# westlake-repl/IDvs.MoRec

Hardware: AMD Instinct MI355X
Metric: user-sequences/sec end-to-end train step, SASRec+BERT-base (higher is better)
Workload: dtype fp16

## Files before the change

### idvs/morec_amd/csrc/gemm8p.hip

```cpp
#include <mutex>
#include "gemm8p_core.hpp"
#include "gemm_args.hpp"
#include "ce_args.hpp"

namespace {
using namespace g8;
constexpr int SLICE = 4096;
constexpr int LDS_TOTAL = LDS_BYTES + 8 * SLICE;

#define G8_STAMPW(i, w)                                                                                  \
    do {                                                                                                 \
        if (p.stamps && threadIdx.x == 0) p.stamps[(size_t)(w) * 16 + (i)] = __builtin_readcyclecounter(); \
    } while (0)

struct TileXY {
    int wg, m0, n0;
    int k0, nkt, tail, chunk;
    int krem;
};

template <typename TI, typename TO, int ACT, bool CS, int TMR = 256>
__device__ __forceinline__ void tile_body(const GemmArgs& p, char* smem, const bf16* __restrict__ Acur, const bf16* __restrict__ Bcur,
                                          const bf16* __restrict__ Anext, const bf16* __restrict__ Bnext, const TileXY cur, const TileXY nxt,
                                          const bool first) {
    constexpr bool PART = TMR != TM;
    constexpr int tmr = TMR;
    constexpr int nb1 = (TMR - 128) / 32;
    constexpr int ES = (int)sizeof(TO);
    constexpr int EPV = 16 / ES;
    constexpr int PC = 128 / ES;
    constexpr int NPASS = 64 / PC;
    constexpr int NG = PC / 8;
    struct Vecs { u32x4_t q[4]; };
    const int m0 = cur.m0, n0 = cur.n0;
    G8_STAMPW(0, cur.wg);
    f32x16_t acc[4][2];
    float bias_l;
    {
        int tid_m = threadIdx.x;
        asm volatile("" : "+v"(tid_m));
        {
            const float* bp = p.bias ? p.bias : reinterpret_cast<const float*>(p.B);
            bias_l = bp[min(n0 + ((tid_m >> 6) & 3) * 64 + (tid_m & 63), p.N - 1)];
        }
        Ctx c;
        make_ctx(c, tid_m, Acur, Bcur, min(p.M - m0, tmr), p.N - n0, p.lda, p.ldb, cur.krem);
        if (first) issue_prologue(c, smem, cur.nkt);
        constexpr int NST = 16 * (int)sizeof(TO) / 2;
        const int younger = (first || (p.debug & 3) || (p.debug & 64)) ? 0 : (p.aux_out ? 2 * NST : NST);
        const int wr_m = __builtin_amdgcn_readfirstlane(tid_m >> 8);
        unsigned long long* st_m = p.stamps ? p.stamps + (size_t)cur.wg * 16 : nullptr;
        if constexpr (!PART) {
            mainloop8p<TI>(c, wr_m, cur.nkt, younger, smem, acc, st_m);
        } else {
            (void)younger;
            if (wr_m == 0) mainloop8p_s<TI, 0, 0, 4>(c, 0, cur.nkt, smem, acc, st_m);
            else mainloop8p_s<TI, 0, 0, nb1>(c, 1, cur.nkt, smem, acc, st_m);
        }
    }
    G8_STAMPW(1, cur.wg);
    if (cur.tail >= 0) {
        int tid_t = threadIdx.x;
        asm volatile("" : "+v"(tid_t));
        const __amdgpu_buffer_rsrc_t rw = __builtin_amdgcn_make_buffer_rsrc((void*)(p.tail_ws + (size_t)(cur.tail * 2 + cur.chunk) * (TM * TN)), 0,
                                                                            TM * TN * 4, 0x00020000);
#pragma unroll
        for (int i = 0; i < 4; ++i)
#pragma unroll
            for (int j = 0; j < 2; ++j)
#pragma unroll
                for (int g = 0; g < 4; ++g) {
                    u32x4_t v;
#pragma unroll
                    for (int e = 0; e < 4; ++e) v[e] = __float_as_uint(acc[i][j][4 * g + e]);
                    __builtin_amdgcn_raw_buffer_store_b128(v, rw, tid_t * 16, ((i * 2 + j) * 4 + g) * (THREADS * 16), 16);
                }
        vm_wait<0>();
        __syncthreads();
        int* flag = reinterpret_cast<int*>(smem + LDS_BYTES);
        if (threadIdx.x == 0) *flag = __hip_atomic_fetch_add(p.tail_cnt + cur.tail, 1, __ATOMIC_RELAXED, __HIP_MEMORY_SCOPE_AGENT);
        __syncthreads();
        const int ticket = __builtin_amdgcn_readfirstlane(*flag);
        __syncthreads();
        if (ticket == 0) return;
        if (threadIdx.x == 0) __hip_atomic_store(p.tail_cnt + cur.tail, 0, __ATOMIC_RELAXED, __HIP_MEMORY_SCOPE_AGENT);
        const __amdgpu_buffer_rsrc_t rr = __builtin_amdgcn_make_buffer_rsrc((void*)(p.tail_ws + (size_t)(cur.tail * 2 + (cur.chunk ^ 1)) * (TM * TN)), 0,
                                                                            TM * TN * 4, 0x00020000);
#pragma unroll
        for (int i = 0; i < 4; ++i) {
            u32x4_t v[2][4];
#pragma unroll
            for (int j = 0; j < 2; ++j)
#pragma unroll
                for (int g = 0; g < 4; ++g) v[j][g] = __builtin_amdgcn_raw_buffer_load_b128(rr, tid_t * 16, ((i * 2 + j) * 4 + g) * (THREADS * 16), 16);
#pragma unroll
            for (int j = 0; j < 2; ++j)
#pragma unroll
                for (int g = 0; g < 4; ++g)
#pragma unroll
                    for (int e = 0; e < 4; ++e) acc[i][j][4 * g + e] += __uint_as_float(v[j][g][e]);
            pin();
        }
    }
    int tid_e = threadIdx.x;
    asm volatile("" : "+v"(tid_e));
    const int lane = tid_e & 63, r5 = lane & 31, h = lane >> 5;
    const int wave = __builtin_amdgcn_readfirstlane(tid_e >> 6);
    const int wr = wave >> 2, wc = wave & 3;
    char* ws = smem + LDS_BYTES + wave * SLICE;
    TO* C = reinterpret_cast<TO*>(p.C);
    TO* aux = reinterpret_cast<TO*>(p.aux_out);
    const TO* din = reinterpret_cast<const TO*>(p.dact_in);
    auto wfence = [&]() {
        __builtin_amdgcn_fence(__ATOMIC_RELEASE, "wavefront");
        __builtin_amdgcn_wave_barrier();
        __builtin_amdgcn_fence(__ATOMIC_ACQUIRE, "wavefront");
    };
    const int rs_row = lane >> 3, rs_slot = lane & 7;
    const int rs_off = rs_row * 128 + ((rs_slot ^ (rs_row & 7)) << 4);
    auto cell = [&](int q) {
        const int slot = ES == 2 ? q : 2 * q + h;
        return reinterpret_cast<TO*>(ws + r5 * 128 + ((slot ^ (r5 & 7)) << 4) + (ES == 2 ? 8 * h : 0));
    };
    const int cur_tm = m0 / tmr;
    const int mw = m0 + wr * 128, nw = n0 + wc * 64;
    const int m_end = min(p.M, m0 + tmr);
    const int nblk = (PART && wr) ? nb1 : 4;
    const long tile_bytes = (long)min(tmr, p.M - m0) * p.ldc * ES;
    const int ext = (int)min(tile_bytes, 0x7fffffffL);
    const size_t tile_off = (size_t)m0 * p.ldc;
    const __amdgpu_buffer_rsrc_t rC = __builtin_amdgcn_make_buffer_rsrc((void*)(C + tile_off), 0, ext, 0x00020000);
    const __amdgpu_buffer_rsrc_t rD = __builtin_amdgcn_make_buffer_rsrc((void*)(((ACT >= 3) ? din : C) + tile_off), 0, ext, 0x00020000);
    auto lane_off = [&](int ps) {
        const int n = nw + ps * PC + rs_slot * EPV;
        return n < p.N ? (uint32_t)((rs_row * p.ldc + n) * ES) : 0x80000000u;
    };
    auto row_term = [&](int Mi, int i) { return (uint32_t)((wr * 128 + Mi * 32 + 8 * i) * p.ldc * ES); };
    auto rows_store = [&](const __amdgpu_buffer_rsrc_t& rs, int Mi, uint32_t lo) {
        u32x4_t q[4];
#pragma unroll
        for (int i = 0; i < 4; ++i) q[i] = *reinterpret_cast<const u32x4_t*>(ws + rs_off + i * 1024);
        if (!(p.debug & 1)) {
            const int cp = (p.debug >> 4) & 3;
            if (cp == 0) {
#pragma unroll
                for (int i = 0; i < 4; ++i) __builtin_amdgcn_raw_buffer_store_b128(q[i], rs, lo + row_term(Mi, i), 0, 0);
            } else if (cp == 1) {
#pragma unroll
                for (int i = 0; i < 4; ++i) __builtin_amdgcn_raw_buffer_store_b128(q[i], rs, lo + row_term(Mi, i), 0, 2);
            } else if (cp == 2) {
#pragma unroll
                for (int i = 0; i < 4; ++i) __builtin_amdgcn_raw_buffer_store_b128(q[i], rs, lo + row_term(Mi, i), 0, 16);
            } else {
#pragma unroll
                for (int i = 0; i < 4; ++i) __builtin_amdgcn_raw_buffer_store_b128(q[i], rs, lo + row_term(Mi, i), 0, 18);
            }
        }
    };
    auto rows_fetch = [&](const __amdgpu_buffer_rsrc_t& rs, int Mi, uint32_t lo) {
        Vecs r;
#pragma unroll
        for (int i = 0; i < 4; ++i) r.q[i] = __builtin_amdgcn_raw_buffer_load_b128(rs, lo + row_term(Mi, i), 0, 0);
        return r;
    };
    auto rows_put = [&](const Vecs r) {
#pragma unroll
        for (int i = 0; i < 4; ++i) *reinterpret_cast<u32x4_t*>(ws + rs_off + i * 1024) = r.q[i];
    };
    uint32_t lo[NPASS];
#pragma unroll
    for (int ps = 0; ps < NPASS; ++ps) lo[ps] = lane_off(ps);

    float4 bv[2][4];
    if constexpr (ACT < 3) {
        reinterpret_cast<float*>(ws)[lane] = p.bias ? bias_l : 0.f;
        wfence();
#pragma unroll
        for (int Ni = 0; Ni < 2; ++Ni)
#pragma unroll
            for (int g = 0; g < 4; ++g) bv[Ni][g] = *reinterpret_cast<const float4*>(ws + (Ni * 32 + g * 8 + 4 * h) * 4);
        wfence();
    } else {
#pragma unroll
        for (int Ni = 0; Ni < 2; ++Ni)
#pragma unroll
            for (int g = 0; g < 4; ++g) bv[Ni][g] = make_float4(0.f, 0.f, 0.f, 0.f);
    }
    Vecs dq[2] = {Vecs(), Vecs()};
    if constexpr (ACT >= 3) {
        dq[0] = rows_fetch(rD, 0, lo[0]);
        dq[1] = rows_fetch(rD, 1 / NPASS, lo[1 % NPASS]);
    }
    pin();

    {
        int tid_n = threadIdx.x;
        asm volatile("" : "+v"(tid_n));
        Ctx cn;
        make_ctx(cn, tid_n, Anext, Bnext, min(p.M - nxt.m0, tmr), p.N - nxt.n0, p.lda, p.ldb, nxt.krem);
        issue_prologue(cn, smem, nxt.nkt);
    }
    if (p.debug & 2) {
        if (acc[0][0][0] == 12345.678f) reinterpret_cast<float*>(p.C)[0] = acc[1][1][3] + acc[2][0][7] + acc[3][1][15] + bv[0][0].x;
        return;
    }
    if (p.stamps) { asm volatile("" :: "v"(bv[0][0].x), "v"(bv[1][3].w)); G8_STAMPW(2, cur.wg); }
    [[maybe_unused]] float cs8[8] = {0.f, 0.f, 0.f, 0.f, 0.f, 0.f, 0.f, 0.f};
#pragma unroll
    for (int Mi = 0; Mi < 4; ++Mi) {
        if constexpr (PART) {
            if (Mi >= nblk) break;
        }
        [[maybe_unused]] const bool row_ok = (mw + Mi * 32 + r5) < m_end;
#pragma unroll
        for (int ps = 0; ps < NPASS; ++ps) {
            pin();
            if constexpr (ACT >= 3) {
                constexpr int LAST = 4 * NPASS - 1;
                const int it = Mi * NPASS + ps, nx = it + 2;
                rows_put(dq[it & 1]);
                if (nx <= LAST) dq[it & 1] = rows_fetch(rD, nx / NPASS, lo[nx % NPASS]);
                wfence();
            }
            if (aux) {
                if constexpr (ACT == 1 || ACT == 2) {
                    static_assert(ES == 2, "activation epilogues are instantiated for bf16 outputs");
                    uint2 park[NG];
#pragma unroll
                    for (int q = 0; q < NG; ++q) {
                        const int Ni = q / 4, g = q % 4;
                        const float4 b = bv[Ni][g];
                        float v[4], d[4];
                        v[0] = fmaf(acc[Mi][Ni][4 * g + 0], p.alpha, b.x);
                        v[1] = fmaf(acc[Mi][Ni][4 * g + 1], p.alpha, b.y);
                        v[2] = fmaf(acc[Mi][Ni][4 * g + 2], p.alpha, b.z);
                        v[3] = fmaf(acc[Mi][Ni][4 * g + 3], p.alpha, b.w);
#pragma unroll
                        for (int r = 0; r < 4; ++r) d[r] = v[r];
                        if (p.aux_deriv) {
                            if constexpr (ACT == 1) {
                                gelu4_with_deriv(v, d);
                            } else {
#pragma unroll
                                for (int r = 0; r < 4; ++r) { d[r] = v[r] > 0.f ? 1.f : 0.f; v[r] = fmaxf(v[r], 0.f); }
                            }
                        } else {
                            if constexpr (ACT == 1) {
                                gelu4(v);
                            } else {
#pragma unroll
                                for (int r = 0; r < 4; ++r) v[r] = fmaxf(v[r], 0.f);
                            }
                        }
                        io<TO>::store4(cell(q), d);
                        park[q] = make_uint2(h16<TI>::pack2(v[0], v[1]), h16<TI>::pack2(v[2], v[3]));
                        if (q & 1) pin();
                    }
                    wfence();
                    rows_store(__builtin_amdgcn_make_buffer_rsrc((void*)(aux + tile_off), 0, ext, 0x00020000), Mi, lo[ps]);
                    wfence();
#pragma unroll
                    for (int q = 0; q < NG; ++q) *reinterpret_cast<uint2*>(cell(q)) = park[q];
                    wfence();
                    rows_store(rC, Mi, lo[ps]);
                    wfence();
                    continue;
                } else {
#pragma unroll
                    for (int q = 0; q < NG; ++q) {
                        const int Ni = ES == 2 ? q / 4 : ps, g = ES == 2 ? q % 4 : q;
                        const float4 b = bv[Ni][g];
                        float pre[4];
                        pre[0] = fmaf(acc[Mi][Ni][4 * g + 0], p.alpha, b.x);
                        pre[1] = fmaf(acc[Mi][Ni][4 * g + 1], p.alpha, b.y);
                        pre[2] = fmaf(acc[Mi][Ni][4 * g + 2], p.alpha, b.z);
                        pre[3] = fmaf(acc[Mi][Ni][4 * g + 3], p.alpha, b.w);
                        io<TO>::store4(cell(q), pre);
                        if (q & 1) pin();
                    }
                    wfence();
                    rows_store(__builtin_amdgcn_make_buffer_rsrc((void*)(aux + tile_off), 0, ext, 0x00020000), Mi, lo[ps]);
                    wfence();
                }
            }
            [[maybe_unused]] uint32_t uraw[NG][ES == 2 ? 2 : 4];
            if constexpr (ACT >= 3) {
#pragma unroll
                for (int q = 0; q < NG; ++q) {
                    if constexpr (ES == 2) {
                        const uint2 t = *reinterpret_cast<const uint2*>(cell(q));
                        uraw[q][0] = t.x; uraw[q][1] = t.y;
                    } else {
                        const uint4 t = *reinterpret_cast<const uint4*>(cell(q));
                        uraw[q][0] = t.x; uraw[q][1] = t.y; uraw[q][2] = t.z; uraw[q][3] = t.w;
                    }
                }
            }
#pragma unroll
            for (int q = 0; q < NG; ++q) {
                const int Ni = ES == 2 ? q / 4 : ps, g = ES == 2 ? q % 4 : q;
                const float4 b = bv[Ni][g];
                float v[4];
                v[0] = fmaf(acc[Mi][Ni][4 * g + 0], p.alpha, b.x);
                v[1] = fmaf(acc[Mi][Ni][4 * g + 1], p.alpha, b.y);
                v[2] = fmaf(acc[Mi][Ni][4 * g + 2], p.alpha, b.z);
                v[3] = fmaf(acc[Mi][Ni][4 * g + 3], p.alpha, b.w);
                if constexpr (ACT == 1) {
                    gelu4(v);
                } else if constexpr (ACT == 2) {
#pragma unroll
                    for (int r = 0; r < 4; ++r) v[r] = fmaxf(v[r], 0.f);
                } else if constexpr (ACT >= 3) {
                    float u[4];
                    if constexpr (ES == 2) {
                        u[0] = h16<TI>::bits2f(uraw[q][0] & 0xffffu); u[1] = h16<TI>::bits2f(uraw[q][0] >> 16);
                        u[2] = h16<TI>::bits2f(uraw[q][1] & 0xffffu); u[3] = h16<TI>::bits2f(uraw[q][1] >> 16);
                    } else {
#pragma unroll
                        for (int r = 0; r < 4; ++r) u[r] = __uint_as_float(uraw[q][r]);
                    }
                    if constexpr (ACT == 3) {
                        dgelu4_mul(v, u);
                    } else if constexpr (ACT == 4) {
#pragma unroll
                        for (int r = 0; r < 4; ++r) v[r] = (u[r] > 0.f) ? v[r] : 0.f;
                    } else {
#pragma unroll
                        for (int r = 0; r < 4; ++r) v[r] *= u[r];
                    }
                }
                if constexpr (CS) {
#pragma unroll
                    for (int r = 0; r < 4; ++r) v[r] = row_ok ? v[r] : 0.f;
                }
                io<TO>::store4(cell(q), v);
                if (ACT != 5 && (q & 1)) pin();
            }
            wfence();
            if constexpr (CS) {
                static_assert(!CS || ES == 2, "fused column sums: bf16 output only");
                u32x4_t q[4];
#pragma unroll
                for (int i = 0; i < 4; ++i) q[i] = *reinterpret_cast<const u32x4_t*>(ws + rs_off + i * 1024);
#pragma unroll
                for (int i = 0; i < 4; ++i)
#pragma unroll
                    for (int w = 0; w < 4; ++w) {
                        cs8[2 * w] += h16<TI>::bits2f(q[i][w] & 0xffffu);
                        cs8[2 * w + 1] += h16<TI>::bits2f(q[i][w] >> 16);
                    }
                if (!(p.debug & 1)) {
#pragma unroll
                    for (int i = 0; i < 4; ++i) __builtin_amdgcn_raw_buffer_store_b128(q[i], rC, lo[ps] + row_term(Mi, i), 0, 0);
                }
            } else {
                rows_store(rC, Mi, lo[ps]);
            }
            wfence();
        }
        G8_STAMPW(3 + Mi, cur.wg);
    }
    G8_STAMPW(7, cur.wg);
    if constexpr (CS) {
#pragma unroll
        for (int j = 0; j < 8; ++j) {
            cs8[j] += __shfl_xor(cs8[j], 8, 64);
            cs8[j] += __shfl_xor(cs8[j], 16, 64);
            cs8[j] += __shfl_xor(cs8[j], 32, 64);
        }
        if (rs_row == 0) {
            const int n = nw + rs_slot * 8;
            float* dst = p.colsum + (size_t)(cur_tm * 2 + wr) * p.N + n;
#pragma unroll
            for (int j = 0; j < 8; ++j)
                if (n + j < p.N) dst[j] = cs8[j];
        }
    }
}

template <typename TI, typename TO, int ACT, bool CS, int TMR = 256>
__global__ __launch_bounds__(THREADS) void gemm8p_kernel(GemmArgs p) {
    extern __shared__ __attribute__((aligned(16))) char smem[];
    const int nwg = p.tiles_m * p.tiles_n;
    const bf16* A = reinterpret_cast<const bf16*>(p.A);
    const bf16* B = reinterpret_cast<const bf16*>(p.B);
    const int Keff = (p.debug & 4) ? 128 : p.K;
    const int nk = (Keff + KE - 1) / KE;
    const int krem_all = Keff - (nk - 1) * KE;
    const int G = gridDim.x, F = nwg / G, R = nwg - F * G;
    const bool split = p.tail_ws != nullptr && F >= 1 && R >= 1 && 2 * R <= G && nk >= 24;
    const int nk0 = (nk + p.tail_bias) / 2;
    const int n_units = F + ((int)blockIdx.x < (split ? 2 * R : R) ? 1 : 0);
    auto unit_at = [&](int i) {
        TileXY t;
        int vb = (int)blockIdx.x + i * G;
        t.k0 = 0; t.nkt = nk; t.tail = -1; t.chunk = 0; t.krem = krem_all;
        if (i >= F && split) {
            t.chunk = (int)blockIdx.x >= R ? 1 : 0;
            t.tail = (int)blockIdx.x - t.chunk * R;
            vb = F * G + t.tail;
            t.k0 = t.chunk ? nk0 : 0;
            t.nkt = t.chunk ? nk - nk0 : nk0;
            t.krem = t.chunk ? krem_all : KE;
        }
        t.wg = xcd_remap(vb, nwg);
        int tm, tn;
        if (p.ngroup <= 0 || p.ngroup >= p.tiles_n) {
            tm = t.wg / p.tiles_n;
            tn = t.wg % p.tiles_n;
        } else {
            const int per = p.ngroup * p.tiles_m, ng = (p.tiles_n + p.ngroup - 1) / p.ngroup;
            const int g = min(t.wg / per, ng - 1), r = t.wg - g * per;
            const int w = g == ng - 1 ? p.tiles_n - g * p.ngroup : p.ngroup;
            tm = r / w;
            tn = g * p.ngroup + r % w;
        }
        t.m0 = tm * TMR;
        t.n0 = tn * TN;
        return t;
    };
    TileXY cur = unit_at(0);
    if (p.debug >> 8) {
        const int GS = (p.debug >> 8) & 0xff;
        const long long T = (long long)nk * 2300 + 9000;
        const long long until = (long long)__builtin_readcyclecounter() + T * ((blockIdx.x >> 3) % GS) / GS;
        while ((long long)__builtin_readcyclecounter() < until) __builtin_amdgcn_s_sleep(16);
    }
    for (int i = 0; i < n_units; ++i) {
        const bool more = i + 1 < n_units;
        const TileXY nxt = more ? unit_at(i + 1) : cur;
        tile_body<TI, TO, ACT, CS, TMR>(p, smem, A + (size_t)cur.m0 * p.lda + cur.k0 * KE, B + (size_t)cur.n0 * p.ldb + cur.k0 * KE,
                               A + (size_t)nxt.m0 * p.lda + nxt.k0 * KE, B + (size_t)nxt.n0 * p.ldb + nxt.k0 * KE, cur, nxt, i == 0);
        cur = nxt;
    }
    vm_wait<0>();
}

static void tail_workspace(hipStream_t s, int n_cu, GemmArgs& a) {
    struct Slot { hipStream_t s; float* ws; int* cnt; int dev; };
    static Slot slots[8];
    static int n_slots = 0;
    static std::mutex mu;
    std::lock_guard<std::mutex> lock(mu);
    int dev = 0;
    (void)hipGetDevice(&dev);
    for (int i = 0; i < n_slots; ++i)
        if (slots[i].s == s && slots[i].dev == dev) { a.tail_ws = slots[i].ws; a.tail_cnt = slots[i].cnt; return; }
    if (n_slots == 8) return;
    const size_t ws_bytes = (size_t)n_cu * TM * TN * sizeof(float), cnt_bytes = (size_t)n_cu * sizeof(int);
    char* base = nullptr;
    if (hipMalloc(reinterpret_cast<void**>(&base), ws_bytes + cnt_bytes) != hipSuccess) { (void)hipGetLastError(); return; }
    if (hipMemset(base + ws_bytes, 0, cnt_bytes) != hipSuccess) { (void)hipGetLastError(); (void)hipFree(base); return; }
    slots[n_slots] = Slot{s, reinterpret_cast<float*>(base), reinterpret_cast<int*>(base + ws_bytes), dev};
    a.tail_ws = slots[n_slots].ws;
    a.tail_cnt = slots[n_slots].cnt;
    ++n_slots;
}

static_assert(TM == gplan::P8_TM && TN == gplan::P8_TN && KE == gplan::P8_KE, "gemm_plan.hpp");

template <typename TI, typename TO, int ACT, bool CS, int TMR = 256>
int launch8p(const GemmPlan& p, GemmArgs& a, hipStream_t s) {
    a.tmr = TMR;
    a.tiles_m = (a.M + TMR - 1) / TMR;
    a.tiles_n = (a.N + TN - 1) / TN;
    static const hipError_t attr_rc = hipFuncSetAttribute(reinterpret_cast<const void*>(&gemm8p_kernel<TI, TO, ACT, CS, TMR>),
                                                          hipFuncAttributeMaxDynamicSharedMemorySize, LDS_TOTAL);
    (void)attr_rc;
    const int n_cu = p.n_cu;
    const int nwg = a.tiles_m * a.tiles_n;
    a.ngroup = p.ngroup;
    a.tail_ws = nullptr;
    a.tail_cnt = nullptr;
    if (p.tail_split) tail_workspace(s, n_cu, a);
    hipLaunchKernelGGL((gemm8p_kernel<TI, TO, ACT, CS, TMR>), dim3(nwg < n_cu ? nwg : n_cu), dim3(THREADS), LDS_TOTAL, s, a);
    MOREC_CHECK_LAUNCH();
    if constexpr (CS) return colsum_f32_launch(a.colsum, a.colsum_dst, a.tiles_m * 2, a.N, s);
    return MOREC_OK;
}

template <typename TI>
int dispatch8p(const GemmPlan& p, GemmArgs& a, hipStream_t s) {
    const int mode = p.mode;
    if (p.tile_rows == 224) {
        if (mode == 0) return launch8p<TI, TI, 0, false, 224>(p, a, s);
        if (mode == 1) return launch8p<TI, TI, 1, false, 224>(p, a, s);
        return launch8p<TI, TI, 5, true, 224>(p, a, s);
    }
    if (p.tile_rows == 192) {
        if (mode == 0) return launch8p<TI, TI, 0, false, 192>(p, a, s);
        if (mode == 1) return launch8p<TI, TI, 1, false, 192>(p, a, s);
        return launch8p<TI, TI, 5, true, 192>(p, a, s);
    }
    if (p.out_dtype == MOREC_F32) return launch8p<TI, float, 0, false>(p, a, s);
    if (p.colsum) {
        if (mode == 3) return launch8p<TI, TI, 3, true>(p, a, s);
        if (mode == 4) return launch8p<TI, TI, 4, true>(p, a, s);
        return launch8p<TI, TI, 5, true>(p, a, s);
    }
    switch (mode) {
        case 1: return launch8p<TI, TI, 1, false>(p, a, s);
        case 2: return launch8p<TI, TI, 2, false>(p, a, s);
        case 3: return launch8p<TI, TI, 3, false>(p, a, s);
        case 4: return launch8p<TI, TI, 4, false>(p, a, s);
        case 5: return launch8p<TI, TI, 5, false>(p, a, s);
        default: return launch8p<TI, TI, 0, false>(p, a, s);
    }
}
}

int gemm8p_launch(const GemmPlan& p, GemmArgs& a, hipStream_t s) {
    const Tuning& t = tuning();
    a.debug = t.gemm8p_debug;
    a.tail_bias = t.gemm8p_tail_bias;
    a.tail_split = t.gemm8p_tail_split;
    a.stamps = reinterpret_cast<unsigned long long*>(t.gemm8p_stamps());
    return p.in_dtype == MOREC_F16 ? dispatch8p<f16>(p, a, s) : dispatch8p<bf16>(p, a, s);
}
```

### idvs/morec_amd/csrc/gemm8p_core.hpp

```cpp
#pragma once
#include "gemm_core.hpp"

namespace g8 {
typedef f32x16c_t f32x16_t;
typedef __attribute__((ext_vector_type(4))) unsigned int u32x4_t;

constexpr int TM = 256, TN = 256, KE = 64;
constexpr int KB = 128;
constexpr int OP_BYTES = 256 * KB;
constexpr int BUF_BYTES = 2 * OP_BYTES;
constexpr int LDS_BYTES = 2 * BUF_BYTES;
constexpr int THREADS = 512;

template <int N>
__device__ __forceinline__ void vm_wait() {
    asm volatile("s_waitcnt vmcnt(%0)" ::"n"(N) : "memory");
}
__device__ __forceinline__ void pin() { __builtin_amdgcn_sched_barrier(0); }
__device__ __forceinline__ void bar() {
    pin();
    __builtin_amdgcn_s_barrier();
    pin();
}

typedef __attribute__((address_space(8))) void* rsrc_t;

template <int AUX = 0>
__device__ __forceinline__ void dma2(__amdgpu_buffer_rsrc_t rs, uint32_t o0, uint32_t o1, int kbyte, char* dst) {
    __builtin_amdgcn_raw_ptr_buffer_load_lds(rs, (lptr_t)dst, 16, o0, kbyte, 0, AUX);
    __builtin_amdgcn_raw_ptr_buffer_load_lds(rs, (lptr_t)(dst + 1024), 16, o1, kbyte, 0, AUX);
}
struct Ctx;
template <int AUX = 0>
__device__ __forceinline__ void dma2z(__amdgpu_buffer_rsrc_t rs, uint32_t o0, uint32_t o1, const uint32_t (&pz)[2], uint32_t m, int kbyte, char* dst) {
    dma2<AUX>(rs, o0 | (pz[0] & m), o1 | (pz[1] & m), kbyte, dst);
}

struct Ctx {
    __amdgpu_buffer_rsrc_t ra, rb;
    uint32_t a1[2], a2[2], b1[2], b2[2];
    int dA1, dA2, dB1, dB2;
    int aoff, boff;
    int loff[4];
    uint32_t pz[2];
};

__device__ __forceinline__ uint4 lds16(const char* p) { return *reinterpret_cast<const uint4*>(p); }

template <typename T16, int M0, int NQ, bool ZERO, int NBW = 4>
__device__ __forceinline__ void mfma_quadrant(f32x16_t (&acc)[4][2], const uint4 (&fa)[2][4], const uint4 (&fb)[4]) {
    if constexpr (M0 >= NBW) return;
    constexpr int NMI = (M0 + 1 < NBW) ? 2 : 1;
#ifndef G8_NO_SETPRIO
    __builtin_amdgcn_s_setprio(1);
#endif
#pragma unroll
    for (int ks = 0; ks < 4; ++ks)
#pragma unroll
        for (int mi = 0; mi < NMI; ++mi) {
            f32x16_t cin = acc[M0 + mi][NQ];
            if constexpr (ZERO) {
                if (ks == 0) {
#pragma unroll
                    for (int v = 0; v < 16; ++v) cin[v] = 0.f;
                }
            }
            acc[M0 + mi][NQ] = h16<T16>::mma32(__builtin_bit_cast(bf16x8_t, fb[ks]), __builtin_bit_cast(bf16x8_t, fa[mi][ks]), cin);
        }
#ifndef G8_NO_SETPRIO
    __builtin_amdgcn_s_setprio(0);
#endif
}

template <int REM, int W1, int W0, int SLACK = 0>
__device__ __forceinline__ void vm_wait_tail() {
    vm_wait<(REM >= 2 ? 8 + SLACK : (REM == 1 ? W1 : W0))>();
}

#ifdef G8_EXP_SHADOW
#define G8_GS_PARAM , float (&gs)[4]
#define G8_GS_ARG , gs
#ifndef G8_EXP_SHADOW_MASK
#define G8_EXP_SHADOW_MASK 15
#endif
#define G8_SHADOW() G8_SHADOW_P(0)
#define G8_SHADOW_P(ph_)                                              \
    do {                                                              \
        if (!((G8_EXP_SHADOW_MASK >> (ph_)) & 1)) break;              \
        pin();                                                        \
        _Pragma("unroll") for (int u_ = 0; u_ < G8_EXP_SHADOW; ++u_) { \
            float d_[4];                                              \
            gelu4_with_deriv(gs, d_);                                 \
            _Pragma("unroll") for (int r_ = 0; r_ < 4; ++r_) gs[r_] = gs[r_] * 0.5f + d_[r_]; \
        }                                                             \
        pin();                                                        \
    } while (0)
#else
#define G8_GS_PARAM
#define G8_GS_ARG
#define G8_SHADOW() do {} while (0)
#define G8_SHADOW_P(ph_) do {} while (0)
#endif
template <typename T16, int REM, int SLACK = 0, bool ZERO = false, int BAUX = 0, int NBW = 4>
__device__ __forceinline__ void ktile(char* smem, const Ctx& c, int cb, int kb, f32x16_t (&acc)[4][2], bool last2 G8_GS_PARAM) {
    const uint32_t m1 = REM == 1 ? 0xffffffffu : 0u;
    const uint32_t m2 = last2 ? 0xffffffffu : 0u;
    static_assert(SLACK == 0 || REM == 2, "slack only on a steady K-tile");
    char* cur = smem + cb;
    char* oth = smem + (cb ^ BUF_BYTES);
    uint4 fa[2][4], fb0[4], fb1[4];
    int ada[4], adb[4];
#pragma unroll
    for (int ks = 0; ks < 4; ++ks) {
        ada[ks] = cb + c.aoff + c.loff[ks];
        adb[ks] = cb + OP_BYTES + c.boff + c.loff[ks];
    }
#pragma unroll
    for (int ks = 0; ks < 4; ++ks) fb0[ks] = lds16(smem + adb[ks]);
#pragma unroll
    for (int mi = 0; mi < 2; ++mi)
#pragma unroll
        for (int ks = 0; ks < 4; ++ks) fa[mi][ks] = lds16(smem + ada[ks] + mi * (32 * KB));
    if constexpr (REM >= 1) dma2z<BAUX>(c.rb, c.b2[0], c.b2[1], c.pz, m1, kb + KB, oth + OP_BYTES + c.dB2);
    G8_SHADOW_P(0);
    pin();
    vm_wait_tail<REM, 8, 2, SLACK>();
    bar();
    mfma_quadrant<T16, 0, 0, ZERO, NBW>(acc, fa, fb0);
    bar();
#pragma unroll
    for (int ks = 0; ks < 4; ++ks) fb1[ks] = lds16(smem + adb[ks] + 32 * KB);
    if constexpr (REM >= 1) dma2z(c.ra, c.a2[0], c.a2[1], c.pz, m1, kb + KB, oth + c.dA2);
    G8_SHADOW_P(1);
    pin();
    vm_wait_tail<REM, 8, 0, SLACK>();
    bar();
    mfma_quadrant<T16, 0, 1, ZERO, NBW>(acc, fa, fb1);
    bar();
#pragma unroll
    for (int mi = 0; mi < 2; ++mi)
#pragma unroll
        for (int ks = 0; ks < 4; ++ks) fa[mi][ks] = lds16(smem + ada[ks] + (64 + mi * 32) * KB);
    if constexpr (REM >= 2) dma2z(c.ra, c.a1[0], c.a1[1], c.pz, m2, kb + 2 * KB, cur + c.dA1);
    G8_SHADOW_P(2);
    pin();
    vm_wait_tail<REM, 6, 0, SLACK>();
    bar();
    mfma_quadrant<T16, 2, 1, ZERO, NBW>(acc, fa, fb1);
    bar();
    if constexpr (REM >= 2) dma2z<BAUX>(c.rb, c.b1[0], c.b1[1], c.pz, m2, kb + 2 * KB, cur + OP_BYTES + c.dB1);
    G8_SHADOW_P(3);
    pin();
    vm_wait_tail<REM, 4, 0, SLACK>();
    bar();
    mfma_quadrant<T16, 2, 0, ZERO, NBW>(acc, fa, fb0);
    bar();
}

__device__ __forceinline__ void make_ctx(Ctx& c, int tid, const bf16* At, const bf16* Bt, int rows_a, int rows_b, int lda, int ldb, int krem) {
    const int lane = tid & 63;
    const int wave = __builtin_amdgcn_readfirstlane(tid >> 6);
    const int wr = wave >> 2, wc = wave & 3;
    const int ra = wr * 128 + wc * 16;
    const int rb = (wave >> 1) * 64 + (wave & 1) * 16;
#pragma unroll
    for (int j = 0; j < 2; ++j) {
        const int rl = j * 8 + (lane >> 3);
        const int slot = (lane & 7) ^ ((rl >> 1) & 7);
        c.a1[j] = (uint32_t)min(ra + rl, rows_a - 1) * (uint32_t)(lda * 2) + slot * 16;
        c.a2[j] = (uint32_t)min(ra + 64 + rl, rows_a - 1) * (uint32_t)(lda * 2) + slot * 16;
        c.b1[j] = (uint32_t)min(rb + rl, rows_b - 1) * (uint32_t)(ldb * 2) + slot * 16;
        c.b2[j] = (uint32_t)min(rb + 32 + rl, rows_b - 1) * (uint32_t)(ldb * 2) + slot * 16;
        c.pz[j] = slot * 8 >= krem ? 0x80000000u : 0u;
    }
    const long abytes = (long)min(256, rows_a) * lda * 2, bbytes = (long)min(256, rows_b) * ldb * 2;
    c.ra = __builtin_amdgcn_make_buffer_rsrc((void*)At, 0, (int)min(abytes, 0x7fffffffL), 0x00020000);
    c.rb = __builtin_amdgcn_make_buffer_rsrc((void*)Bt, 0, (int)min(bbytes, 0x7fffffffL), 0x00020000);
    c.dA1 = ra * KB; c.dA2 = (ra + 64) * KB; c.dB1 = rb * KB; c.dB2 = (rb + 32) * KB;
    c.aoff = wr * 128 * KB;
    c.boff = wc * 64 * KB;
    const int r5 = lane & 31, fr = (r5 >> 1) & 7;
#pragma unroll
    for (int ks = 0; ks < 4; ++ks) c.loff[ks] = r5 * KB + (((2 * ks + (lane >> 5)) ^ fr) << 4);
}

template <int BAUX = 0>
__device__ __forceinline__ void issue_prologue(const Ctx& c, char* smem, int nk) {
    const uint32_t m = nk == 2 ? 0xffffffffu : 0u;
    dma2(c.ra, c.a1[0], c.a1[1], 0, smem + c.dA1);
    dma2<BAUX>(c.rb, c.b1[0], c.b1[1], 0, smem + OP_BYTES + c.dB1);
    dma2<BAUX>(c.rb, c.b2[0], c.b2[1], 0, smem + OP_BYTES + c.dB2);
    dma2(c.ra, c.a2[0], c.a2[1], 0, smem + c.dA2);
    dma2z(c.ra, c.a1[0], c.a1[1], c.pz, m, KB, smem + BUF_BYTES + c.dA1);
    dma2z<BAUX>(c.rb, c.b1[0], c.b1[1], c.pz, m, KB, smem + BUF_BYTES + OP_BYTES + c.dB1);
    pin();
}

#define G8_MSTAMP(i)                                                                    \
    do {                                                                                \
        if (st && threadIdx.x == 0) st[(i)] = __builtin_readcyclecounter();              \
    } while (0)
template <typename T16, int SLACK, int BAUX = 0, int NBW = 4>
__device__ __forceinline__ void mainloop8p_s(const Ctx& c, int wr, int nk, char* smem, f32x16_t (&acc)[4][2], unsigned long long* st) {
    G8_MSTAMP(8);
    vm_wait<8 + SLACK>();
    G8_MSTAMP(9);
    bar();
    if (wr == 1) bar();
    G8_MSTAMP(10);
#ifdef G8_EXP_SHADOW
    float gs[4];
#pragma unroll
    for (int r = 0; r < 4; ++r) gs[r] = (float)(c.loff[r] & 255) * 0.01f;
#endif
    int cb = 0;
    int t = 0;
    if (nk >= 3) {
        ktile<T16, 2, SLACK, true, BAUX, NBW>(smem, c, cb, 0, acc, nk == 3 G8_GS_ARG);
        cb ^= BUF_BYTES;
        t = 1;
    } else {
#pragma unroll
        for (int i = 0; i < 4; ++i)
#pragma unroll
            for (int j = 0; j < 2; ++j)
#pragma unroll
                for (int v = 0; v < 16; ++v) acc[i][j][v] = 0.f;
    }
    G8_MSTAMP(11);
    for (; t < nk - 2; ++t) {
        ktile<T16, 2, 0, false, BAUX, NBW>(smem, c, cb, t * KB, acc, t + 3 == nk G8_GS_ARG);
        cb ^= BUF_BYTES;
        if (t == 1) G8_MSTAMP(12);
    }
    G8_MSTAMP(13);
    ktile<T16, 1, 0, false, BAUX, NBW>(smem, c, cb, t * KB, acc, false G8_GS_ARG);
    ktile<T16, 0, 0, false, BAUX, NBW>(smem, c, cb ^ BUF_BYTES, (t + 1) * KB, acc, false G8_GS_ARG);
#ifdef G8_EXP_SHADOW
    asm volatile("" ::"v"(gs[0]), "v"(gs[1]), "v"(gs[2]), "v"(gs[3]));
#endif
    G8_MSTAMP(14);
    if (wr == 0) bar();
    G8_MSTAMP(15);
}
template <typename T16, int BAUX = 0>
__device__ __forceinline__ void mainloop8p(const Ctx& c, int wr, int nk, int younger, char* smem, f32x16_t (&acc)[4][2],
                                           unsigned long long* st) {
    if (younger >= 32) mainloop8p_s<T16, 32, BAUX>(c, wr, nk, smem, acc, st);
    else if (younger >= 16) mainloop8p_s<T16, 16, BAUX>(c, wr, nk, smem, acc, st);
    else mainloop8p_s<T16, 0, BAUX>(c, wr, nk, smem, acc, st);
}
}
```

### idvs/morec_amd/csrc/gemm_plan.hpp

```cpp
#pragma once
#include <initializer_list>
#include "morec_hip.h"
#include "tuning.hpp"

enum GemmFamily {
    GEMM_UNSUPPORTED = MOREC_GEMM_UNSUPPORTED,
    GEMM_SKINNY = MOREC_GEMM_SKINNY,
    GEMM_SKINNY_WIDE = MOREC_GEMM_SKINNY_WIDE,
    GEMM_TWO_W = MOREC_GEMM_TWO_W,
    GEMM_EIGHT_P = MOREC_GEMM_EIGHT_P,
    GEMM_SMALL = MOREC_GEMM_SMALL,
    GEMM_GENERIC = MOREC_GEMM_GENERIC,
};
enum GemmGenericTile {
    GEMM_TILE_128_W8,
    GEMM_TILE_256_W16,
    GEMM_TILE_128_W4,
    GEMM_TILE_256_W8,
    GEMM_TILE_256x128,
};

namespace gplan {
constexpr int P8_TM = 256, P8_TN = 256, P8_KE = 64;
constexpr int W2_TM = 256, W2_TN = 128, W2_KE = 64;
constexpr int SK_TR = 32;
constexpr int SMALL_T = 64;
inline bool is16(int dtype) { return dtype == MOREC_BF16 || dtype == MOREC_F16; }
}

struct GemmOperands {
    bool bias, aux_out, dact_in, colsum;
    bool vec_store;
    bool bias_aligned16;
};

struct GemmPlan {
    int family;
    int error;
    int in_dtype, out_dtype;
    int mode;
    int colsum;
    int tile_rows, tile_cols;
    int ngroup;
    int tail_split;
    int n_cu;
    int nbh, ksteps;
    int generic_tile;
    int split_k;
    int wave_epilogue;
};

inline int gemm_epilogue_mode(int act, int dact) {
    return dact == MOREC_ACT_GELU ? 3 : dact == MOREC_ACT_RELU ? 4 : dact == MOREC_DACT_MUL ? 5
           : act == MOREC_ACT_GELU ? 1 : act == MOREC_ACT_RELU ? 2 : 0;
}

inline int pick_tmr(int tmr_mode, int M, int tiles_n, int nk, int n_cu) {
    using namespace gplan;
    if (tmr_mode == 0) return P8_TM;
    if (tmr_mode == 224 || tmr_mode == 192) return tmr_mode;
    const double fixed = 4.0;
    int best = P8_TM;
    double best_cost = 0.0;
    for (int t : {256, 224, 192}) {
        const long tiles = (long)((M + t - 1) / t) * tiles_n;
        if (tiles <= n_cu && t != P8_TM) continue;
        const double cost = (double)((tiles + n_cu - 1) / n_cu) * ((double)nk * t / 256.0 + fixed);
        if (t == P8_TM || cost < best_cost * 0.985) { if (t == P8_TM || cost < best_cost) { best = t; best_cost = cost; } }
    }
    return best;
}

inline GemmPlan gemm_plan(const morec_gemm_desc& d, const GemmOperands& o, const Tuning& t, int n_cu) {
    using namespace gplan;
    GemmPlan p{};
    p.in_dtype = d.in_dtype;
    p.out_dtype = d.out_dtype;
    p.mode = gemm_epilogue_mode(d.act, d.dact);
    p.colsum = o.colsum;
    p.split_k = d.split_k < 1 ? 1 : d.split_k;
    p.wave_epilogue = t.gemm_epi == 2 ? ((o.aux_out || d.N <= 1024) ? 1 : 0) : t.gemm_epi;
    const bool same16 = is16(d.in_dtype) && d.out_dtype == d.in_dtype;
    const bool staged16 = is16(d.in_dtype) && d.accumulate == 0 && o.vec_store && d.split_k <= 1;
    const bool streaming = !o.aux_out && !o.dact_in && !o.colsum && d.dact == MOREC_ACT_NONE && d.accumulate == 0 && d.split_k <= 1 &&
                           d.alpha == 1.0f && !(o.bias && (d.N % 4 || !o.bias_aligned16)) && d.lda % 8 == 0 && d.ldb % 8 == 0 && d.ldc % 8 == 0 &&
                           d.N % 8 == 0 && d.K % 8 == 0 && d.M >= 8192 && (long)SK_TR * d.lda * 2 < 0x7fffffffL;

    if (t.gemm_skinny != 1 && same16 && streaming && d.act == MOREC_ACT_NONE && d.N <= 288 && d.N >= 64 && d.K <= 384 && !(d.N > 128 && d.K > 96)) {
        p.family = GEMM_SKINNY;
        p.nbh = d.N <= 96 ? 3 : (d.N <= 128 ? 4 : 9);
        p.ksteps = (d.K + 31) / 32;
        p.tile_rows = SK_TR;
        p.tile_cols = 32 * p.nbh;
        return p;
    }
    if (t.gemm_skinny != 1 && t.gemm_skinny != 2 && same16 && streaming && d.act == MOREC_ACT_GELU && d.N > 288 && d.N <= 768 && d.K <= 192 &&
        d.K >= 32 && (long)SK_TR * d.ldc * 2 < 0x7fffffffL) {
        p.family = GEMM_SKINNY_WIDE;
        p.tile_rows = SK_TR;
        p.tile_cols = d.N;
        return p;
    }
    if (t.gemm2w != 1 && same16 && staged16 && d.K % W2_KE == 0 && d.K >= W2_KE && d.N % 8 == 0 && d.M >= 1 &&
        (d.dact == MOREC_ACT_NONE || d.dact == MOREC_DACT_MUL) && !(d.dact == MOREC_DACT_MUL && o.bias) && d.act != MOREC_ACT_RELU &&
        !(o.aux_out && d.act != MOREC_ACT_GELU) && !(o.colsum && (d.dact != MOREC_DACT_MUL || d.M < 128))) {
        const int tiles_m = (d.M + W2_TM - 1) / W2_TM, tiles_n = (d.N + W2_TN - 1) / W2_TN;
        const long waste = (long)((d.N + 255) / 256) * 256 - d.N;
        const bool narrow = p.mode == 0 && !o.colsum && waste * 4 >= d.N && d.M >= 8192 && d.K <= 2048;
        const bool dmul = p.mode == 5 && d.M >= 16384 && ((d.M <= 40000 && d.K <= 768) || (d.M <= 70000 && d.K <= 512));
        if ((long)tiles_m * tiles_n >= 64 && (t.gemm2w == 2 || narrow || dmul)) {
            p.family = GEMM_TWO_W;
            p.tile_rows = W2_TM;
            p.tile_cols = W2_TN;
            p.ngroup = tiles_n <= 8 ? 0 : 8;
            return p;
        }
    }
    if (t.gemm8p != 1 && staged16 && d.K % 8 == 0 && d.K > P8_KE && d.N >= 64 && d.M >= 1 && !(o.colsum && d.M < 128) &&
        !(d.dact != MOREC_ACT_NONE && o.bias) &&
        (d.out_dtype == d.in_dtype ? !(o.colsum && p.mode < 3) : (d.out_dtype == MOREC_F32 && p.mode == 0 && !o.colsum))) {
        const int tiles_n = (d.N + P8_TN - 1) / P8_TN;
        const long tiles = (long)((d.M + P8_TM - 1) / P8_TM) * tiles_n;
        if (t.gemm8p == 2 || !(tiles < (d.K >= 2048 ? 160 : 192) || tiles_n * P8_TN * 100L > d.N * 134L)) {
            p.family = GEMM_EIGHT_P;
            p.n_cu = n_cu;
            p.tile_rows = P8_TM;
            if (d.out_dtype == d.in_dtype && ((p.mode == 0 && !o.colsum) || (p.mode == 1 && !o.colsum) || (p.mode == 5 && o.colsum)))
                p.tile_rows = pick_tmr(t.gemm8p_tmr, d.M, tiles_n, (d.K + P8_KE - 1) / P8_KE, n_cu);
            p.tile_cols = P8_TN;
            const int ng = (tiles_n + 5) / 6;
            p.ngroup = t.gemm8p_ngroup < 0 ? (tiles_n + ng - 1) / ng : t.gemm8p_ngroup;
            const long nwg = (long)((d.M + p.tile_rows - 1) / p.tile_rows) * tiles_n;
            p.tail_split = p.tile_rows == P8_TM && t.gemm8p_tail_split && nwg > n_cu && nwg % n_cu && 2 * (nwg % n_cu) <= n_cu &&
                           d.K >= 24 * P8_KE && !(t.gemm8p_debug & 128);
            return p;
        }
    }
    if (t.gemm_small != 1 && same16 && staged16 && d.K >= 64 && d.M >= 1) {
        const long t128 = (long)((d.M + 127) / 128) * ((d.N + 127) / 128);
        if (t.gemm_small == 2 || !(t128 > 128 || d.K < 1024 || d.N < 256 || o.aux_out || o.colsum)) {
            if (o.colsum && p.mode < 3) { p.error = MOREC_E_UNSUPPORTED; return p; }
            p.family = GEMM_SMALL;
            p.tile_rows = p.tile_cols = SMALL_T;
            p.wave_epilogue = 1;
            return p;
        }
    }
    if (!((d.in_dtype == MOREC_F32 && d.out_dtype == MOREC_F32) || (is16(d.in_dtype) && (d.out_dtype == d.in_dtype || d.out_dtype == MOREC_F32)))) {
        p.error = MOREC_E_DTYPE;
        return p;
    }
    if (o.colsum && p.mode < 3) { p.error = MOREC_E_UNSUPPORTED; return p; }
    p.family = GEMM_GENERIC;
    const long big_tiles = (long)((d.M + 255) / 256) * ((d.N + 255) / 256) * p.split_k;
    if (t.gemm_tile == 128) p.generic_tile = GEMM_TILE_128_W4;
    else if (t.gemm_tile == 256) p.generic_tile = GEMM_TILE_256_W8;
    else if (t.gemm_tile == 129) p.generic_tile = GEMM_TILE_128_W8;
    else if (t.gemm_tile == 2128) p.generic_tile = GEMM_TILE_256x128;
    else if (t.gemm_tile == 1024) p.generic_tile = GEMM_TILE_256_W16;
    else if (d.N <= 128 || d.K <= 96) p.generic_tile = GEMM_TILE_128_W8;
    else if (big_tiles >= 192) p.generic_tile = GEMM_TILE_256_W16;
    else p.generic_tile = GEMM_TILE_128_W8;
    p.tile_rows = (p.generic_tile == GEMM_TILE_128_W8 || p.generic_tile == GEMM_TILE_128_W4) ? 128 : 256;
    p.tile_cols = p.generic_tile == GEMM_TILE_256x128 ? 128 : p.tile_rows;
    return p;
}
```

### idvs/morec_amd/csrc/tuning.hip

```cpp
#include <stdlib.h>
#include <string.h>
#include "common.hpp"

namespace {
enum Handling {
    RAW,
    FLAG,
    TMR,
    RESERVE,
    TAIL_BIAS,
    AT_LEAST_1,
    NOT_CHAR_0,
    IS_CHAR_1,
    EPI,
};
struct Row {
    const char* key;
    const char* env;
    int Tuning::*field;
    int def;
    Handling how;
};
const Row ROWS[] = {
    {"gemm8p", "MOREC_GEMM8P", &Tuning::gemm8p, 0, RAW},
    {"gemm2w", "MOREC_GEMM2W", &Tuning::gemm2w, 0, RAW},
    {"gemm_small", "MOREC_GEMM_SMALL", &Tuning::gemm_small, 0, RAW},
    {"gemm_skinny", "MOREC_GEMM_SKINNY", &Tuning::gemm_skinny, 0, RAW},
    {"ce8p", "MOREC_CE8P", &Tuning::ce8p, 0, RAW},
    {"gemm8p_tmr", "MOREC_GEMM8P_TMR", &Tuning::gemm8p_tmr, 1, TMR},
    {"gemm8p_ngroup", "MOREC_GEMM8P_NGROUP", &Tuning::gemm8p_ngroup, -1, RAW},
    {"gemm8p_reserve_cus", "MOREC_GEMM8P_RESERVE_CUS", &Tuning::gemm8p_reserve_cus, 0, RESERVE},
    {"gemm8p_tail_split", "MOREC_GEMM8P_TAIL_SPLIT", &Tuning::gemm8p_tail_split, 0, FLAG},
    {"gemm8p_tail_bias", nullptr, &Tuning::gemm8p_tail_bias, 2, TAIL_BIAS},
    {"gemm8p_debug", "MOREC_GEMM8P_DEBUG", &Tuning::gemm8p_debug, 0, RAW},
    {"gemm8p_stamps_lo", nullptr, &Tuning::gemm8p_stamps_lo, 0, RAW},
    {"gemm8p_stamps_hi", nullptr, &Tuning::gemm8p_stamps_hi, 0, RAW},
    {"deterministic", "MOREC_DETERMINISTIC", &Tuning::deterministic, 0, FLAG},
    {"fold_defer", "MOREC_FOLD_DEFER", &Tuning::fold_defer, 1, FLAG},
    {nullptr, "MOREC_GEMM_TILE", &Tuning::gemm_tile, 0, RAW},
    {nullptr, "MOREC_GEMM_EPI", &Tuning::gemm_epi, 2, EPI},
    {nullptr, "MOREC_GEMM2W_STAGGER", &Tuning::gemm2w_stagger, 0, RAW},
    {nullptr, "MOREC_TN8P_SKIP", &Tuning::tn8p_skip, 1, FLAG},
    {nullptr, "MOREC_ATTN_MFMA64", &Tuning::attn_mfma64, 1, NOT_CHAR_0},
    {nullptr, "MOREC_ATTN_F32_MFMA", &Tuning::attn_f32_mfma, 1, NOT_CHAR_0},
    {nullptr, "MOREC_SWIN_WPW_MIN", &Tuning::swin_wpw_min, 8, AT_LEAST_1},
    {nullptr, "MOREC_SWIN_BWD_WIDE", &Tuning::swin_bwd_wide, 1, RAW},
    {nullptr, "MOREC_QUIET", &Tuning::quiet, 0, IS_CHAR_1},
};

int handled(Handling how, int v) {
    switch (how) {
        case FLAG: return v != 0;
        case TMR: return (v == 0 || v == 1 || v == 224 || v == 192) ? v : 1;
        case RESERVE: return v < 0 ? 0 : v > 128 ? 128 : v;
        case TAIL_BIAS: return v < 0 ? 0 : v > 16 ? 16 : v;
        case AT_LEAST_1: return v < 1 ? 1 : v;
        default: return v;
    }
}

Tuning& table() {
    static Tuning t = [] {
        Tuning x{};
        for (const Row& r : ROWS) {
            const char* e = r.env ? getenv(r.env) : nullptr;
            x.*r.field = !e                    ? r.def
                         : r.how == NOT_CHAR_0 ? e[0] != '0'
                         : r.how == IS_CHAR_1  ? e[0] == '1'
                         : r.how == EPI        ? e[0] == 'w'
                                               : handled(r.how, atoi(e));
        }
        return x;
    }();
    return t;
}
}

const Tuning& tuning() { return table(); }

extern "C" int morec_tuning_set(const char* key, int value) {
    if (!key) return MOREC_E_ARG;
    for (const Row& r : ROWS)
        if (r.key && !strcmp(key, r.key)) {
            table().*r.field = handled(r.how, value);
            return MOREC_OK;
        }
    return MOREC_E_UNSUPPORTED;
}

bool morec_deterministic() { return tuning().deterministic != 0; }
void morec_set_deterministic(int on) { table().deterministic = on ? 1 : 0; }

int device_cu_count() {
    static const int n = [] {
        int dev = 0, c = 0;
        (void)hipGetDevice(&dev);
        if (hipDeviceGetAttribute(&c, hipDeviceAttributeMultiprocessorCount, dev) != hipSuccess || c <= 0) c = 256;
        return c;
    }();
    return n;
}

int gemm8p_cu_count() {
    const int n_dev = device_cu_count() & ~7;
    const int n = (n_dev < 8 ? 8 : n_dev) - (tuning().gemm8p_reserve_cus & ~7);
    return n < 8 ? 8 : n;
}
```

### idvs/morec_amd/csrc/tuning.hpp

```cpp
#pragma once

struct Tuning {
    int gemm8p, gemm2w, gemm_small, gemm_skinny, ce8p;
    int gemm8p_tmr;
    int gemm8p_ngroup;
    int gemm8p_reserve_cus;
    int gemm8p_tail_split, gemm8p_tail_bias;
    int gemm8p_debug;
    int gemm8p_stamps_lo, gemm8p_stamps_hi;
    int deterministic;
    int fold_defer;
    int gemm_tile;
    int gemm_epi;
    int gemm2w_stagger;
    int tn8p_skip;
    int attn_mfma64;
    int attn_f32_mfma;
    int swin_wpw_min;
    int swin_bwd_wide;
    int quiet;

    unsigned long long gemm8p_stamps() const {
        return ((unsigned long long)(unsigned)gemm8p_stamps_hi << 32) | (unsigned)gemm8p_stamps_lo;
    }
};

const Tuning& tuning();

int device_cu_count();
int gemm8p_cu_count();
```

Baseline: 3620.

## Add 16x16 MFMA variant to gemm8p kernel and make it the default

Templates the gemm8p mainloop, fragment LDS addressing and epilogue on the MFMA shape. A new 16x16x32 path issues four smaller MFMAs per 32x32 block, with remapped LDS offsets, bias and row-guard indexing. The planner selects 16 by default, overridable through MOREC_GEMM8P_MFMA. The smaller shape may give better instruction issue or latency behaviour on MI355X, at the cost of more MFMA instructions per tile and a new layout mapping that must match the accumulator order exactly.

```diff
diff --git a/idvs/morec_amd/csrc/gemm8p.hip b/idvs/morec_amd/csrc/gemm8p.hip
--- a/idvs/morec_amd/csrc/gemm8p.hip
+++ b/idvs/morec_amd/csrc/gemm8p.hip
@@ -19,7 +19,15 @@
     int krem;
 };
 
-template <typename TI, typename TO, int ACT, bool CS, int TMR = 256>
+template <int MF, int ES>
+struct Grp {
+    static constexpr int ni(int q, int ps) { return ES == 2 ? (MF == 32 ? q / 4 : (q & 3) >> 1) : ps; }
+    static constexpr int e0(int q) { return MF == 32 ? 4 * (ES == 2 ? q % 4 : q) : 4 * (ES == 2 ? 2 * (q >> 2) + (q & 1) : q); }
+    static constexpr int bi(int q) { return MF == 32 ? (ES == 2 ? q % 4 : q) : (q & 1); }
+    static constexpr int half(int q) { return MF == 32 ? 0 : (ES == 2 ? q >> 2 : q >> 1); }
+};
+
+template <typename TI, typename TO, int ACT, bool CS, int TMR = 256, int MF = 32>
 __device__ __forceinline__ void tile_body(const GemmArgs& p, char* smem, const bf16* __restrict__ Acur, const bf16* __restrict__ Bcur,
                                           const bf16* __restrict__ Anext, const bf16* __restrict__ Bnext, const TileXY cur, const TileXY nxt,
                                           const bool first) {
@@ -31,6 +39,7 @@
     constexpr int PC = 128 / ES;
     constexpr int NPASS = 64 / PC;
     constexpr int NG = PC / 8;
+    using G = Grp<MF, ES>;
     struct Vecs { u32x4_t q[4]; };
     const int m0 = cur.m0, n0 = cur.n0;
     G8_STAMPW(0, cur.wg);
@@ -44,18 +53,18 @@
             bias_l = bp[min(n0 + ((tid_m >> 6) & 3) * 64 + (tid_m & 63), p.N - 1)];
         }
         Ctx c;
-        make_ctx(c, tid_m, Acur, Bcur, min(p.M - m0, tmr), p.N - n0, p.lda, p.ldb, cur.krem);
+        make_ctx<MF>(c, tid_m, Acur, Bcur, min(p.M - m0, tmr), p.N - n0, p.lda, p.ldb, cur.krem);
         if (first) issue_prologue(c, smem, cur.nkt);
         constexpr int NST = 16 * (int)sizeof(TO) / 2;
         const int younger = (first || (p.debug & 3) || (p.debug & 64)) ? 0 : (p.aux_out ? 2 * NST : NST);
         const int wr_m = __builtin_amdgcn_readfirstlane(tid_m >> 8);
         unsigned long long* st_m = p.stamps ? p.stamps + (size_t)cur.wg * 16 : nullptr;
         if constexpr (!PART) {
-            mainloop8p<TI>(c, wr_m, cur.nkt, younger, smem, acc, st_m);
+            mainloop8p<TI, 0, MF>(c, wr_m, cur.nkt, younger, smem, acc, st_m);
         } else {
             (void)younger;
-            if (wr_m == 0) mainloop8p_s<TI, 0, 0, 4>(c, 0, cur.nkt, smem, acc, st_m);
-            else mainloop8p_s<TI, 0, 0, nb1>(c, 1, cur.nkt, smem, acc, st_m);
+            if (wr_m == 0) mainloop8p_s<TI, 0, 0, 4, MF>(c, 0, cur.nkt, smem, acc, st_m);
+            else mainloop8p_s<TI, 0, 0, nb1, MF>(c, 1, cur.nkt, smem, acc, st_m);
         }
     }
     G8_STAMPW(1, cur.wg);
@@ -104,7 +113,7 @@
     }
     int tid_e = threadIdx.x;
     asm volatile("" : "+v"(tid_e));
-    const int lane = tid_e & 63, r5 = lane & 31, h = lane >> 5;
+    const int lane = tid_e & 63, r5 = MF == 32 ? lane & 31 : lane & 15, h = MF == 32 ? lane >> 5 : lane >> 4;
     const int wave = __builtin_amdgcn_readfirstlane(tid_e >> 6);
     const int wr = wave >> 2, wc = wave & 3;
     char* ws = smem + LDS_BYTES + wave * SLICE;
@@ -119,8 +128,13 @@
     const int rs_row = lane >> 3, rs_slot = lane & 7;
     const int rs_off = rs_row * 128 + ((rs_slot ^ (rs_row & 7)) << 4);
     auto cell = [&](int q) {
-        const int slot = ES == 2 ? q : 2 * q + h;
-        return reinterpret_cast<TO*>(ws + r5 * 128 + ((slot ^ (r5 & 7)) << 4) + (ES == 2 ? 8 * h : 0));
+        if constexpr (MF == 32) {
+            const int slot = ES == 2 ? q : 2 * q + h;
+            return reinterpret_cast<TO*>(ws + r5 * 128 + ((slot ^ (r5 & 7)) << 4) + (ES == 2 ? 8 * h : 0));
+        } else {
+            const int slot = ES == 2 ? 2 * (q & 3) + (h >> 1) : 4 * (q & 1) + h;
+            return reinterpret_cast<TO*>(ws + (16 * G::half(q) + r5) * 128 + ((slot ^ (r5 & 7)) << 4) + (ES == 2 ? 8 * (h & 1) : 0));
+        }
     };
     const int cur_tm = m0 / tmr;
     const int mw = m0 + wr * 128, nw = n0 + wc * 64;
@@ -178,7 +192,9 @@
 #pragma unroll
         for (int Ni = 0; Ni < 2; ++Ni)
 #pragma unroll
-            for (int g = 0; g < 4; ++g) bv[Ni][g] = *reinterpret_cast<const float4*>(ws + (Ni * 32 + g * 8 + 4 * h) * 4);
+            for (int g = 0; g < 4; ++g)
+                bv[Ni][g] = (MF == 32 || g < 2) ? *reinterpret_cast<const float4*>(ws + (Ni * 32 + g * (MF == 32 ? 8 : 16) + 4 * h) * 4)
+                                                : make_float4(0.f, 0.f, 0.f, 0.f);
         wfence();
     } else {
 #pragma unroll
@@ -197,7 +213,7 @@
         int tid_n = threadIdx.x;
         asm volatile("" : "+v"(tid_n));
         Ctx cn;
-        make_ctx(cn, tid_n, Anext, Bnext, min(p.M - nxt.m0, tmr), p.N - nxt.n0, p.lda, p.ldb, nxt.krem);
+        make_ctx<MF>(cn, tid_n, Anext, Bnext, min(p.M - nxt.m0, tmr), p.N - nxt.n0, p.lda, p.ldb, nxt.krem);
         issue_prologue(cn, smem, nxt.nkt);
     }
     if (p.debug & 2) {
@@ -211,7 +227,7 @@
         if constexpr (PART) {
             if (Mi >= nblk) break;
         }
-        [[maybe_unused]] const bool row_ok = (mw + Mi * 32 + r5) < m_end;
+        [[maybe_unused]] const bool row_ok[2] = {(mw + Mi * 32 + r5) < m_end, (mw + Mi * 32 + 16 + r5) < m_end};
 #pragma unroll
         for (int ps = 0; ps < NPASS; ++ps) {
             pin();
@@ -228,13 +244,13 @@
                     uint2 park[NG];
 #pragma unroll
                     for (int q = 0; q < NG; ++q) {
-                        const int Ni = q / 4, g = q % 4;
-                        const float4 b = bv[Ni][g];
+                        const int Ni = G::ni(q, ps), e0 = G::e0(q);
+                        const float4 b = bv[Ni][G::bi(q)];
                         float v[4], d[4];
-                        v[0] = fmaf(acc[Mi][Ni][4 * g + 0], p.alpha, b.x);
-                        v[1] = fmaf(acc[Mi][Ni][4 * g + 1], p.alpha, b.y);
-                        v[2] = fmaf(acc[Mi][Ni][4 * g + 2], p.alpha, b.z);
-                        v[3] = fmaf(acc[Mi][Ni][4 * g + 3], p.alpha, b.w);
+                        v[0] = fmaf(acc[Mi][Ni][e0 + 0], p.alpha, b.x);
+                        v[1] = fmaf(acc[Mi][Ni][e0 + 1], p.alpha, b.y);
+                        v[2] = fmaf(acc[Mi][Ni][e0 + 2], p.alpha, b.z);
+                        v[3] = fmaf(acc[Mi][Ni][e0 + 3], p.alpha, b.w);
 #pragma unroll
                         for (int r = 0; r < 4; ++r) d[r] = v[r];
                         if (p.aux_deriv) {
@@ -268,13 +284,13 @@
                 } else {
 #pragma unroll
                     for (int q = 0; q < NG; ++q) {
-                        const int Ni = ES == 2 ? q / 4 : ps, g = ES == 2 ? q % 4 : q;
-                        const float4 b = bv[Ni][g];
+                        const int Ni = G::ni(q, ps), e0 = G::e0(q);
+                        const float4 b = bv[Ni][G::bi(q)];
                         float pre[4];
-                        pre[0] = fmaf(acc[Mi][Ni][4 * g + 0], p.alpha, b.x);
-                        pre[1] = fmaf(acc[Mi][Ni][4 * g + 1], p.alpha, b.y);
-                        pre[2] = fmaf(acc[Mi][Ni][4 * g + 2], p.alpha, b.z);
-                        pre[3] = fmaf(acc[Mi][Ni][4 * g + 3], p.alpha, b.w);
+                        pre[0] = fmaf(acc[Mi][Ni][e0 + 0], p.alpha, b.x);
+                        pre[1] = fmaf(acc[Mi][Ni][e0 + 1], p.alpha, b.y);
+                        pre[2] = fmaf(acc[Mi][Ni][e0 + 2], p.alpha, b.z);
+                        pre[3] = fmaf(acc[Mi][Ni][e0 + 3], p.alpha, b.w);
                         io<TO>::store4(cell(q), pre);
                         if (q & 1) pin();
                     }
@@ -298,13 +314,13 @@
             }
 #pragma unroll
             for (int q = 0; q < NG; ++q) {
-                const int Ni = ES == 2 ? q / 4 : ps, g = ES == 2 ? q % 4 : q;
-                const float4 b = bv[Ni][g];
+                const int Ni = G::ni(q, ps), e0 = G::e0(q);
+                const float4 b = bv[Ni][G::bi(q)];
                 float v[4];
-                v[0] = fmaf(acc[Mi][Ni][4 * g + 0], p.alpha, b.x);
-                v[1] = fmaf(acc[Mi][Ni][4 * g + 1], p.alpha, b.y);
-                v[2] = fmaf(acc[Mi][Ni][4 * g + 2], p.alpha, b.z);
-                v[3] = fmaf(acc[Mi][Ni][4 * g + 3], p.alpha, b.w);
+                v[0] = fmaf(acc[Mi][Ni][e0 + 0], p.alpha, b.x);
+                v[1] = fmaf(acc[Mi][Ni][e0 + 1], p.alpha, b.y);
+                v[2] = fmaf(acc[Mi][Ni][e0 + 2], p.alpha, b.z);
+                v[3] = fmaf(acc[Mi][Ni][e0 + 3], p.alpha, b.w);
                 if constexpr (ACT == 1) {
                     gelu4(v);
                 } else if constexpr (ACT == 2) {
@@ -331,7 +347,7 @@
                 }
                 if constexpr (CS) {
 #pragma unroll
-                    for (int r = 0; r < 4; ++r) v[r] = row_ok ? v[r] : 0.f;
+                    for (int r = 0; r < 4; ++r) v[r] = row_ok[G::half(q)] ? v[r] : 0.f;
                 }
                 io<TO>::store4(cell(q), v);
                 if (ACT != 5 && (q & 1)) pin();
@@ -378,7 +394,7 @@
     }
 }
 
-template <typename TI, typename TO, int ACT, bool CS, int TMR = 256>
+template <typename TI, typename TO, int ACT, bool CS, int TMR = 256, int MF = 32>
 __global__ __launch_bounds__(THREADS) void gemm8p_kernel(GemmArgs p) {
     extern __shared__ __attribute__((aligned(16))) char smem[];
     const int nwg = p.tiles_m * p.tiles_n;
@@ -429,7 +445,7 @@
     for (int i = 0; i < n_units; ++i) {
         const bool more = i + 1 < n_units;
         const TileXY nxt = more ? unit_at(i + 1) : cur;
-        tile_body<TI, TO, ACT, CS, TMR>(p, smem, A + (size_t)cur.m0 * p.lda + cur.k0 * KE, B + (size_t)cur.n0 * p.ldb + cur.k0 * KE,
+        tile_body<TI, TO, ACT, CS, TMR, MF>(p, smem, A + (size_t)cur.m0 * p.lda + cur.k0 * KE, B + (size_t)cur.n0 * p.ldb + cur.k0 * KE,
                                A + (size_t)nxt.m0 * p.lda + nxt.k0 * KE, B + (size_t)nxt.n0 * p.ldb + nxt.k0 * KE, cur, nxt, i == 0);
         cur = nxt;
     }
@@ -459,12 +475,12 @@
 
 static_assert(TM == gplan::P8_TM && TN == gplan::P8_TN && KE == gplan::P8_KE, "gemm_plan.hpp");
 
-template <typename TI, typename TO, int ACT, bool CS, int TMR = 256>
+template <typename TI, typename TO, int ACT, bool CS, int TMR = 256, int MF = 32>
 int launch8p(const GemmPlan& p, GemmArgs& a, hipStream_t s) {
     a.tmr = TMR;
     a.tiles_m = (a.M + TMR - 1) / TMR;
     a.tiles_n = (a.N + TN - 1) / TN;
-    static const hipError_t attr_rc = hipFuncSetAttribute(reinterpret_cast<const void*>(&gemm8p_kernel<TI, TO, ACT, CS, TMR>),
+    static const hipError_t attr_rc = hipFuncSetAttribute(reinterpret_cast<const void*>(&gemm8p_kernel<TI, TO, ACT, CS, TMR, MF>),
                                                           hipFuncAttributeMaxDynamicSharedMemorySize, LDS_TOTAL);
     (void)attr_rc;
     const int n_cu = p.n_cu;
@@ -473,38 +489,38 @@
     a.tail_ws = nullptr;
     a.tail_cnt = nullptr;
     if (p.tail_split) tail_workspace(s, n_cu, a);
-    hipLaunchKernelGGL((gemm8p_kernel<TI, TO, ACT, CS, TMR>), dim3(nwg < n_cu ? nwg : n_cu), dim3(THREADS), LDS_TOTAL, s, a);
+    hipLaunchKernelGGL((gemm8p_kernel<TI, TO, ACT, CS, TMR, MF>), dim3(nwg < n_cu ? nwg : n_cu), dim3(THREADS), LDS_TOTAL, s, a);
     MOREC_CHECK_LAUNCH();
     if constexpr (CS) return colsum_f32_launch(a.colsum, a.colsum_dst, a.tiles_m * 2, a.N, s);
     return MOREC_OK;
 }
 
-template <typename TI>
+template <typename TI, int MF>
 int dispatch8p(const GemmPlan& p, GemmArgs& a, hipStream_t s) {
     const int mode = p.mode;
     if (p.tile_rows == 224) {
-        if (mode == 0) return launch8p<TI, TI, 0, false, 224>(p, a, s);
-        if (mode == 1) return launch8p<TI, TI, 1, false, 224>(p, a, s);
-        return launch8p<TI, TI, 5, true, 224>(p, a, s);
+        if (mode == 0) return launch8p<TI, TI, 0, false, 224, MF>(p, a, s);
+        if (mode == 1) return launch8p<TI, TI, 1, false, 224, MF>(p, a, s);
+        return launch8p<TI, TI, 5, true, 224, MF>(p, a, s);
     }
     if (p.tile_rows == 192) {
-        if (mode == 0) return launch8p<TI, TI, 0, false, 192>(p, a, s);
-        if (mode == 1) return launch8p<TI, TI, 1, false, 192>(p, a, s);
-        return launch8p<TI, TI, 5, true, 192>(p, a, s);
-    }
-    if (p.out_dtype == MOREC_F32) return launch8p<TI, float, 0, false>(p, a, s);
+        if (mode == 0) return launch8p<TI, TI, 0, false, 192, MF>(p, a, s);
+        if (mode == 1) return launch8p<TI, TI, 1, false, 192, MF>(p, a, s);
+        return launch8p<TI, TI, 5, true, 192, MF>(p, a, s);
+    }
+    if (p.out_dtype == MOREC_F32) return launch8p<TI, float, 0, false, 256, MF>(p, a, s);
     if (p.colsum) {
-        if (mode == 3) return launch8p<TI, TI, 3, true>(p, a, s);
-        if (mode == 4) return launch8p<TI, TI, 4, true>(p, a, s);
-        return launch8p<TI, TI, 5, true>(p, a, s);
+        if (mode == 3) return launch8p<TI, TI, 3, true, 256, MF>(p, a, s);
+        if (mode == 4) return launch8p<TI, TI, 4, true, 256, MF>(p, a, s);
+        return launch8p<TI, TI, 5, true, 256, MF>(p, a, s);
     }
     switch (mode) {
-        case 1: return launch8p<TI, TI, 1, false>(p, a, s);
-        case 2: return launch8p<TI, TI, 2, false>(p, a, s);
-        case 3: return launch8p<TI, TI, 3, false>(p, a, s);
-        case 4: return launch8p<TI, TI, 4, false>(p, a, s);
-        case 5: return launch8p<TI, TI, 5, false>(p, a, s);
-        default: return launch8p<TI, TI, 0, false>(p, a, s);
+        case 1: return launch8p<TI, TI, 1, false, 256, MF>(p, a, s);
+        case 2: return launch8p<TI, TI, 2, false, 256, MF>(p, a, s);
+        case 3: return launch8p<TI, TI, 3, false, 256, MF>(p, a, s);
+        case 4: return launch8p<TI, TI, 4, false, 256, MF>(p, a, s);
+        case 5: return launch8p<TI, TI, 5, false, 256, MF>(p, a, s);
+        default: return launch8p<TI, TI, 0, false, 256, MF>(p, a, s);
     }
 }
 }
@@ -515,5 +531,6 @@
     a.tail_bias = t.gemm8p_tail_bias;
     a.tail_split = t.gemm8p_tail_split;
     a.stamps = reinterpret_cast<unsigned long long*>(t.gemm8p_stamps());
-    return p.in_dtype == MOREC_F16 ? dispatch8p<f16>(p, a, s) : dispatch8p<bf16>(p, a, s);
-}
+    if (p.mfma == 16) return p.in_dtype == MOREC_F16 ? dispatch8p<f16, 16>(p, a, s) : dispatch8p<bf16, 16>(p, a, s);
+    return p.in_dtype == MOREC_F16 ? dispatch8p<f16, 32>(p, a, s) : dispatch8p<bf16, 32>(p, a, s);
+}
diff --git a/idvs/morec_amd/csrc/gemm8p_core.hpp b/idvs/morec_amd/csrc/gemm8p_core.hpp
--- a/idvs/morec_amd/csrc/gemm8p_core.hpp
+++ b/idvs/morec_amd/csrc/gemm8p_core.hpp
@@ -47,13 +47,31 @@
 
 __device__ __forceinline__ uint4 lds16(const char* p) { return *reinterpret_cast<const uint4*>(p); }
 
-template <typename T16, int M0, int NQ, bool ZERO, int NBW = 4>
+template <typename T16, int M0, int NQ, bool ZERO, int NBW = 4, int MF = 32>
 __device__ __forceinline__ void mfma_quadrant(f32x16_t (&acc)[4][2], const uint4 (&fa)[2][4], const uint4 (&fb)[4]) {
+    static_assert(MF == 32 || MF == 16, "MFMA shape");
     if constexpr (M0 >= NBW) return;
     constexpr int NMI = (M0 + 1 < NBW) ? 2 : 1;
 #ifndef G8_NO_SETPRIO
     __builtin_amdgcn_s_setprio(1);
 #endif
+    if constexpr (MF == 16) {
+#pragma unroll
+        for (int ks = 0; ks < 2; ++ks)
+#pragma unroll
+            for (int mi = 0; mi < NMI; ++mi)
+#pragma unroll
+                for (int sb = 0; sb < 4; ++sb) {
+                    f32x16_t& blk = acc[M0 + mi][NQ];
+                    f32x4_t cin;
+#pragma unroll
+                    for (int v = 0; v < 4; ++v) cin[v] = (ZERO && ks == 0) ? 0.f : blk[4 * sb + v];
+                    const f32x4_t d = h16<T16>::mma16(__builtin_bit_cast(bf16x8_t, fb[2 * (sb & 1) + ks]),
+                                                      __builtin_bit_cast(bf16x8_t, fa[mi][2 * (sb >> 1) + ks]), cin);
+#pragma unroll
+                    for (int v = 0; v < 4; ++v) blk[4 * sb + v] = d[v];
+                }
+    } else {
 #pragma unroll
     for (int ks = 0; ks < 4; ++ks)
 #pragma unroll
@@ -67,6 +85,7 @@
             }
             acc[M0 + mi][NQ] = h16<T16>::mma32(__builtin_bit_cast(bf16x8_t, fb[ks]), __builtin_bit_cast(bf16x8_t, fa[mi][ks]), cin);
         }
+    }
 #ifndef G8_NO_SETPRIO
     __builtin_amdgcn_s_setprio(0);
 #endif
@@ -101,7 +120,7 @@
 #define G8_SHADOW() do {} while (0)
 #define G8_SHADOW_P(ph_) do {} while (0)
 #endif
-template <typename T16, int REM, int SLACK = 0, bool ZERO = false, int BAUX = 0, int NBW = 4>
+template <typename T16, int REM, int SLACK = 0, bool ZERO = false, int BAUX = 0, int NBW = 4, int MF = 32>
 __device__ __forceinline__ void ktile(char* smem, const Ctx& c, int cb, int kb, f32x16_t (&acc)[4][2], bool last2 G8_GS_PARAM) {
     const uint32_t m1 = REM == 1 ? 0xffffffffu : 0u;
     const uint32_t m2 = last2 ? 0xffffffffu : 0u;
@@ -126,7 +145,7 @@
     pin();
     vm_wait_tail<REM, 8, 2, SLACK>();
     bar();
-    mfma_quadrant<T16, 0, 0, ZERO, NBW>(acc, fa, fb0);
+    mfma_quadrant<T16, 0, 0, ZERO, NBW, MF>(acc, fa, fb0);
     bar();
 #pragma unroll
     for (int ks = 0; ks < 4; ++ks) fb1[ks] = lds16(smem + adb[ks] + 32 * KB);
@@ -135,7 +154,7 @@
     pin();
     vm_wait_tail<REM, 8, 0, SLACK>();
     bar();
-    mfma_quadrant<T16, 0, 1, ZERO, NBW>(acc, fa, fb1);
+    mfma_quadrant<T16, 0, 1, ZERO, NBW, MF>(acc, fa, fb1);
     bar();
 #pragma unroll
     for (int mi = 0; mi < 2; ++mi)
@@ -146,17 +165,18 @@
     pin();
     vm_wait_tail<REM, 6, 0, SLACK>();
     bar();
-    mfma_quadrant<T16, 2, 1, ZERO, NBW>(acc, fa, fb1);
+    mfma_quadrant<T16, 2, 1, ZERO, NBW, MF>(acc, fa, fb1);
     bar();
     if constexpr (REM >= 2) dma2z<BAUX>(c.rb, c.b1[0], c.b1[1], c.pz, m2, kb + 2 * KB, cur + OP_BYTES + c.dB1);
     G8_SHADOW_P(3);
     pin();
     vm_wait_tail<REM, 4, 0, SLACK>();
     bar();
-    mfma_quadrant<T16, 2, 0, ZERO, NBW>(acc, fa, fb0);
-    bar();
-}
-
+    mfma_quadrant<T16, 2, 0, ZERO, NBW, MF>(acc, fa, fb0);
+    bar();
+}
+
+template <int MF = 32>
 __device__ __forceinline__ void make_ctx(Ctx& c, int tid, const bf16* At, const bf16* Bt, int rows_a, int rows_b, int lda, int ldb, int krem) {
     const int lane = tid & 63;
     const int wave = __builtin_amdgcn_readfirstlane(tid >> 6);
@@ -179,9 +199,15 @@
     c.dA1 = ra * KB; c.dA2 = (ra + 64) * KB; c.dB1 = rb * KB; c.dB2 = (rb + 32) * KB;
     c.aoff = wr * 128 * KB;
     c.boff = wc * 64 * KB;
-    const int r5 = lane & 31, fr = (r5 >> 1) & 7;
-#pragma unroll
-    for (int ks = 0; ks < 4; ++ks) c.loff[ks] = r5 * KB + (((2 * ks + (lane >> 5)) ^ fr) << 4);
+    if constexpr (MF == 16) {
+        const int r4 = lane & 15, fr = (r4 >> 1) & 7;
+#pragma unroll
+        for (int e = 0; e < 4; ++e) c.loff[e] = ((e >> 1) * 16 + r4) * KB + (((4 * (e & 1) + (lane >> 4)) ^ fr) << 4);
+    } else {
+        const int r5 = lane & 31, fr = (r5 >> 1) & 7;
+#pragma unroll
+        for (int ks = 0; ks < 4; ++ks) c.loff[ks] = r5 * KB + (((2 * ks + (lane >> 5)) ^ fr) << 4);
+    }
 }
 
 template <int BAUX = 0>
@@ -200,7 +226,7 @@
     do {                                                                                \
         if (st && threadIdx.x == 0) st[(i)] = __builtin_readcyclecounter();              \
     } while (0)
-template <typename T16, int SLACK, int BAUX = 0, int NBW = 4>
+template <typename T16, int SLACK, int BAUX = 0, int NBW = 4, int MF = 32>
 __device__ __forceinline__ void mainloop8p_s(const Ctx& c, int wr, int nk, char* smem, f32x16_t (&acc)[4][2], unsigned long long* st) {
     G8_MSTAMP(8);
     vm_wait<8 + SLACK>();
@@ -216,7 +242,7 @@
     int cb = 0;
     int t = 0;
     if (nk >= 3) {
-        ktile<T16, 2, SLACK, true, BAUX, NBW>(smem, c, cb, 0, acc, nk == 3 G8_GS_ARG);
+        ktile<T16, 2, SLACK, true, BAUX, NBW, MF>(smem, c, cb, 0, acc, nk == 3 G8_GS_ARG);
         cb ^= BUF_BYTES;
         t = 1;
     } else {
@@ -229,13 +255,13 @@
     }
     G8_MSTAMP(11);
     for (; t < nk - 2; ++t) {
-        ktile<T16, 2, 0, false, BAUX, NBW>(smem, c, cb, t * KB, acc, t + 3 == nk G8_GS_ARG);
+        ktile<T16, 2, 0, false, BAUX, NBW, MF>(smem, c, cb, t * KB, acc, t + 3 == nk G8_GS_ARG);
         cb ^= BUF_BYTES;
         if (t == 1) G8_MSTAMP(12);
     }
     G8_MSTAMP(13);
-    ktile<T16, 1, 0, false, BAUX, NBW>(smem, c, cb, t * KB, acc, false G8_GS_ARG);
-    ktile<T16, 0, 0, false, BAUX, NBW>(smem, c, cb ^ BUF_BYTES, (t + 1) * KB, acc, false G8_GS_ARG);
+    ktile<T16, 1, 0, false, BAUX, NBW, MF>(smem, c, cb, t * KB, acc, false G8_GS_ARG);
+    ktile<T16, 0, 0, false, BAUX, NBW, MF>(smem, c, cb ^ BUF_BYTES, (t + 1) * KB, acc, false G8_GS_ARG);
 #ifdef G8_EXP_SHADOW
     asm volatile("" ::"v"(gs[0]), "v"(gs[1]), "v"(gs[2]), "v"(gs[3]));
 #endif
@@ -243,11 +269,11 @@
     if (wr == 0) bar();
     G8_MSTAMP(15);
 }
-template <typename T16, int BAUX = 0>
+template <typename T16, int BAUX = 0, int MF = 32>
 __device__ __forceinline__ void mainloop8p(const Ctx& c, int wr, int nk, int younger, char* smem, f32x16_t (&acc)[4][2],
                                            unsigned long long* st) {
-    if (younger >= 32) mainloop8p_s<T16, 32, BAUX>(c, wr, nk, smem, acc, st);
-    else if (younger >= 16) mainloop8p_s<T16, 16, BAUX>(c, wr, nk, smem, acc, st);
-    else mainloop8p_s<T16, 0, BAUX>(c, wr, nk, smem, acc, st);
-}
-}
+    if (younger >= 32) mainloop8p_s<T16, 32, BAUX, 4, MF>(c, wr, nk, smem, acc, st);
+    else if (younger >= 16) mainloop8p_s<T16, 16, BAUX, 4, MF>(c, wr, nk, smem, acc, st);
+    else mainloop8p_s<T16, 0, BAUX, 4, MF>(c, wr, nk, smem, acc, st);
+}
+}
diff --git a/idvs/morec_amd/csrc/gemm_plan.hpp b/idvs/morec_amd/csrc/gemm_plan.hpp
--- a/idvs/morec_amd/csrc/gemm_plan.hpp
+++ b/idvs/morec_amd/csrc/gemm_plan.hpp
@@ -44,6 +44,7 @@
     int ngroup;
     int tail_split;
     int n_cu;
+    int mfma;
     int nbh, ksteps;
     int generic_tile;
     int split_k;
@@ -128,6 +129,7 @@
             if (d.out_dtype == d.in_dtype && ((p.mode == 0 && !o.colsum) || (p.mode == 1 && !o.colsum) || (p.mode == 5 && o.colsum)))
                 p.tile_rows = pick_tmr(t.gemm8p_tmr, d.M, tiles_n, (d.K + P8_KE - 1) / P8_KE, n_cu);
             p.tile_cols = P8_TN;
+            p.mfma = t.gemm8p_mfma ? t.gemm8p_mfma : 16;
             const int ng = (tiles_n + 5) / 6;
             p.ngroup = t.gemm8p_ngroup < 0 ? (tiles_n + ng - 1) / ng : t.gemm8p_ngroup;
             const long nwg = (long)((d.M + p.tile_rows - 1) / p.tile_rows) * tiles_n;
diff --git a/idvs/morec_amd/csrc/tuning.hip b/idvs/morec_amd/csrc/tuning.hip
--- a/idvs/morec_amd/csrc/tuning.hip
+++ b/idvs/morec_amd/csrc/tuning.hip
@@ -9,6 +9,7 @@
     TMR,
     RESERVE,
     TAIL_BIAS,
+    MFMA,
     AT_LEAST_1,
     NOT_CHAR_0,
     IS_CHAR_1,
@@ -32,6 +33,7 @@
     {"gemm8p_reserve_cus", "MOREC_GEMM8P_RESERVE_CUS", &Tuning::gemm8p_reserve_cus, 0, RESERVE},
     {"gemm8p_tail_split", "MOREC_GEMM8P_TAIL_SPLIT", &Tuning::gemm8p_tail_split, 0, FLAG},
     {"gemm8p_tail_bias", nullptr, &Tuning::gemm8p_tail_bias, 2, TAIL_BIAS},
+    {"gemm8p_mfma", "MOREC_GEMM8P_MFMA", &Tuning::gemm8p_mfma, 0, MFMA},
     {"gemm8p_debug", "MOREC_GEMM8P_DEBUG", &Tuning::gemm8p_debug, 0, RAW},
     {"gemm8p_stamps_lo", nullptr, &Tuning::gemm8p_stamps_lo, 0, RAW},
     {"gemm8p_stamps_hi", nullptr, &Tuning::gemm8p_stamps_hi, 0, RAW},
@@ -54,6 +56,7 @@
         case TMR: return (v == 0 || v == 1 || v == 224 || v == 192) ? v : 1;
         case RESERVE: return v < 0 ? 0 : v > 128 ? 128 : v;
         case TAIL_BIAS: return v < 0 ? 0 : v > 16 ? 16 : v;
+        case MFMA: return (v == 16 || v == 32) ? v : 0;
         case AT_LEAST_1: return v < 1 ? 1 : v;
         default: return v;
     }
@@ -82,6 +85,7 @@
     if (!key) return MOREC_E_ARG;
     for (const Row& r : ROWS)
         if (r.key && !strcmp(key, r.key)) {
+            if (r.how == MFMA && value != 0 && value != 16 && value != 32) return MOREC_E_UNSUPPORTED;
             table().*r.field = handled(r.how, value);
             return MOREC_OK;
         }
diff --git a/idvs/morec_amd/csrc/tuning.hpp b/idvs/morec_amd/csrc/tuning.hpp
--- a/idvs/morec_amd/csrc/tuning.hpp
+++ b/idvs/morec_amd/csrc/tuning.hpp
@@ -6,6 +6,7 @@
     int gemm8p_ngroup;
     int gemm8p_reserve_cus;
     int gemm8p_tail_split, gemm8p_tail_bias;
+    int gemm8p_mfma;
     int gemm8p_debug;
     int gemm8p_stamps_lo, gemm8p_stamps_hi;
     int deterministic;
```

Result: faster. 3684 (median of 6 runs) (+1.8%).
